# Veason-silverbullet/DIGAT

Hardware: AMD Instinct MI355X
Metric: MIND dev impressions scored/sec (AUC match not run) (higher is better)
Workload: dtype f32; 1 GPU; MIND-small default: --graph_encoder=DIGAT neighbors=3 hops=2 (N=10, U=67), d=400, graph_depth=3, fp32 dev inference; projection=auto -> fp16x3, N=10, U=67, d=400, graph_depth=3, news_num=65238, parallelism=dp1 (row shards, no data-path collective), ranks_in_process_group=1

## Files before the change

### digat_amd/_lib.py

```python
from __future__ import annotations

import ctypes as C
import os
from typing import Optional

import torch

_HERE = os.path.dirname(os.path.abspath(__file__))
LIB_PATH = os.environ.get("DIGAT_HIP_LIB") or os.path.join(_HERE, "lib", "libdigat_hip.so")
DIGAT_MAX_DEPTH = 16
DIGAT_MAX_NODES = 128
GEMM_BF16X6, GEMM_F16X3 = 0, 1
GEMM_F16F8C = 2
PARAMS_GEMM_F16X3 = 64
PARAMS_BD_TILED = 128
PARAMS_PQ_FP8 = 256
PARAMS_SIDE_STREAM_OFF, PARAMS_SIDE_STREAM_ON = 512, 1024
PARAMS_NO_LIVE_ROWS = 2048
PARAMS_PROJ_F16F8C = 4096
PARAMS_RAGGED_OFF, PARAMS_RAGGED_ROWMAJOR = 8192, 16384

_f = C.c_void_p


# ... 34 lines not shown
class Params(C.Structure):
    _fields_ = ([("d", C.c_int32), ("depth", C.c_int32), ("category_num", C.c_int32), ("flags", C.c_int32)]
                + [(k, _f) for k in ("topic_node_embedding", "cand_K", "cand_Q", "cand_bQ",
                                     "news_graph_W", "news_graph_b", "user_news_K", "user_news_Q",
                                     "user_news_bQ", "featureAffine_W", "featureAffine_b",
                                     "userAtt_K", "userAtt_Q", "userAtt_bQ")]
                + [("news", LayerParams * DIGAT_MAX_DEPTH), ("user", LayerParams * DIGAT_MAX_DEPTH)]
                + [(k, _f) for k in ("cand_fold_W", "cand_fold_b", "user_news_fold_W", "user_news_fold_b",
                                     "userAtt_fold_W", "userAtt_fold_b", "featureAffine_wsplit", "cand_fold_wsplit", "gate_wsplit")]
                + [("ctx_wsplit", _f * (DIGAT_MAX_DEPTH + 1)), ("range_flag", _f), ("featureAffine_fsplit", _f)])


class DigatHipError(RuntimeError):
    pass


_lib: Optional[C.CDLL] = None

_SIGNATURES = {
    "digat_version": (C.c_int, []),
    "digat_error_string": (C.c_char_p, [C.c_int]),
    "digat_linear_f32": (C.c_int, [_f, C.c_int64, _f, _f, _f, C.c_int64, C.c_int, C.c_int, C.c_int, _f]),
    "digat_xattn_workspace_bytes": (C.c_size_t, [C.c_int] * 3),
    "digat_xattn_fwd": (C.c_int, [_f] * 12 + [C.c_int] * 3 + [_f, C.c_size_t, _f]),
    "digat_xattn_fwd_mode": (C.c_int, [_f] * 11 + [C.c_int] * 4 + [_f, C.c_size_t, _f]),
    "digat_xattn_fwd_lowprec": (C.c_int, [_f] * 11 + [C.c_int, _f] + [C.c_int] * 4 + [_f, C.c_size_t, _f]),
    "digat_xattn_pairwise_fwd": (C.c_int, [_f] * 8 + [C.c_int] * 3 + [_f]),
    "digat_news_ctx_workspace_bytes": (C.c_size_t, [C.c_int] * 3),
    "digat_news_ctx_fwd": (C.c_int, [_f] * 9 + [C.c_int] * 3 + [_f, C.c_size_t, _f]),
    "digat_user_ctx_workspace_bytes": (C.c_size_t, [C.c_int] * 5),
    "digat_user_ctx_fwd": (C.c_int, [_f] * 14 + [C.c_int] * 5 + [_f, C.c_size_t, _f]),
    "digat_user_ctx_grouped_workspace_bytes": (C.c_size_t, [C.c_int] * 6),
    "digat_user_ctx_fwd_grouped": (C.c_int, [_f] * 15 + [C.c_int] * 6 + [_f, C.c_size_t, _f]),
    "digat_user_nodes_build": (C.c_int, [_f] * 4 + [C.c_long, C.c_long] + [C.c_int] * 3 + [_f]),
    "digat_topic_pool_fwd": (C.c_int, [_f] * 4 + [C.c_int] * 5 + [_f]),
    "digat_encoder_workspace_bytes": (C.c_size_t, [C.c_int] * 6),
    "digat_encoder_fwd": (C.c_int, [C.POINTER(Params)] + [_f] * 10 + [C.c_int] * 3 + [_f, C.c_size_t, _f]),
    "digat_row_logits": (C.c_int, [_f] * 3 + [C.c_int] * 2 + [_f]),
    "digat_profile_pause": (C.c_int, [C.c_int]),
    "digat_set_train_precision": (C.c_int, [C.c_int]),
    "digat_gather_tables": (C.c_int, [C.POINTER(GatherJob), C.c_int, _f]),
    "digat_user_graph_build": (C.c_int, [_f, _f, C.c_long, C.c_int, C.c_int, _f, _f, _f, _f]),
    "digat_negative_sample": (C.c_int, [_f, _f, _f, C.c_long, C.c_int, C.c_uint32, C.c_uint32, _f, _f]),
    "digat_train_batch_ids": (C.c_int, [_f, C.c_long, _f, _f, C.c_long, C.c_int, _f, C.c_long, C.c_int, _f, C.c_long, C.c_int, _f, _f, _f, _f, _f]),
    "digat_profile_live_row_fraction": (C.c_double, []),
    "digat_rank_metrics": (C.c_int, [_f] * 3 + [C.c_int] + [_f] * 4),
    "digat_format_rank_file": (C.c_int64, [_f, _f, C.c_int64, _f, C.c_int64]),
    "digat_topk_segments_workspace_bytes": (C.c_size_t, [C.c_int64, C.c_int64, C.c_int]),
    "digat_topk_segments": (C.c_int, [_f, _f, C.c_int64, C.c_int64, _f, _f, C.c_int, C.c_int, _f, _f, _f, _f, C.c_size_t, _f]),
    "digat_dot_topk_workspace_bytes": (C.c_size_t, [C.c_int64, C.c_int64, C.c_int]),
    "digat_dot_topk": (C.c_int, [_f, _f, _f, C.c_int64, C.c_int64, C.c_int64, C.c_int, _f, C.c_int, C.c_int, _f, _f, _f, _f, C.c_size_t, _f]),
    "digat_dot_scores": (C.c_int, [_f, _f, _f, C.c_int64, C.c_int64, C.c_int64, C.c_int, _f, _f]),
    "digat_shortlist_segments_workspace_bytes": (C.c_size_t, [C.c_int64, C.c_int64, C.c_int]),
    "digat_shortlist_segments": (C.c_int, [_f, _f, C.c_int64, C.c_int64, _f, _f, C.c_int, C.c_int, _f, _f, _f, _f, C.c_size_t, _f]),
    "digat_dot_shortlist_workspace_bytes": (C.c_size_t, [C.c_int64, C.c_int64, C.c_int, C.c_int64]),
    "digat_dot_shortlist": (C.c_int, [_f, _f, _f, C.c_int64, C.c_int64, C.c_int64, C.c_int, _f, C.c_int, C.c_int, C.c_int64, _f, _f, _f, _f,
                                      C.c_size_t, _f]),
    "digat_quantize_rows_i8": (C.c_int, [_f, C.c_int64, C.c_int, C.c_int, _f, _f, _f]),
    "digat_qdot_scores": (C.c_int, [_f] * 5 + [C.c_int64] * 3 + [C.c_int, C.c_int, _f, _f]),
    "digat_qdot_topk_workspace_bytes": (C.c_size_t, [C.c_int64, C.c_int64, C.c_int]),
    "digat_qdot_topk": (C.c_int, [_f] * 5 + [C.c_int64] * 3 + [C.c_int, C.c_int, _f, C.c_int, C.c_int, _f, _f, _f, _f, C.c_size_t, _f]),
    "digat_qdot_shortlist_workspace_bytes": (C.c_size_t, [C.c_int64, C.c_int64, C.c_int, C.c_int64]),
    "digat_qdot_shortlist": (C.c_int, [_f] * 5 + [C.c_int64] * 3 + [C.c_int, C.c_int, _f, C.c_int, C.c_int, C.c_int64, _f, _f, _f, _f,
                                       C.c_size_t, _f]),
    "digat_dot_rank_workspace_bytes":(C.c_size_t, [C.c_int64, C.c_int64, C.c_int64]),
    "digat_dot_rank": (C.c_int, [_f, _f, _f, C.c_int64, C.c_int64, C.c_int64, C.c_int, _f, C.c_int, _f, _f, C.c_int64, _f, _f, _f, C.c_size_t, _f]),
# ... 296 lines not shown
```

### digat_amd/csrc/digat_encoder.inc

```
static size_t max_sz(size_t a, size_t b) { return a > b ? a : b; }

struct FoldCtxWs { float *T, *T2, *glob; };
struct EncoderWs {
    float *Xu[2], *Xn[2];
    char* xws; size_t xws_bytes;
    XattnWs xu;
    char* cws; size_t cws_bytes;
    FoldCtxWs fc;
    float *kq_t, *kq_u, *r_user[2], *r_news;
    char* xws_news; size_t xws_news_bytes;
    XattnWs xn;
    int *cnt, *off, *idx, *cnt2, *off2, *idx2, *entries, *flag, *hlast;
    uint8_t *flags1, *flags2;
    int *cnt_n, *off_n, *idx_n; uint8_t* flags_n;
    int *l0_gs, *l0_off; uint8_t* l0_lead; int* l0_idx;
    unsigned* tw_word; int* tw_list; uint8_t* tw_flags; int *tw_cnt, *tw_off;
    int *gl_off, *gl_idx;
    int* idx32;
    uint8_t *Au, *cm; int64_t* ci;
    uint8_t *fg, *tfg; unsigned* twg; uint8_t* bfg; int *cg, *eg, *hg, *bcg, *tcg;
    uint8_t *same, *is_leader, *lead; int* leader_of;
};
static bool encoder_carve(Arena& a, int B, int N, int H, int C, int d, int variant, EncoderWs& e) {
    const int U = H + C, C1 = C + 1, nmax = N > U ? N : U;
// ... 18 lines not shown
    e.flags1 = a.take<uint8_t>(bu); e.flags2 = a.take<uint8_t>(b * C1);
    e.cnt_n = a.take<int>(b); e.off_n = a.take<int>(b + 1); e.idx_n = a.take<int>(b * N); e.flags_n = a.take<uint8_t>(b * N);
    e.l0_gs = a.take<int>(b + 64); e.l0_off = a.take<int>(b + 64); e.l0_lead = a.take<uint8_t>(b); e.l0_idx = a.take<int>(bu);
    e.tw_word = a.take<unsigned>(bu); e.tw_list = a.take<int>(bu); e.tw_flags = a.take<uint8_t>(bu);
    e.tw_cnt = a.take<int>(b + 64); e.tw_off = a.take<int>(b + 64);
    e.gl_off = a.take<int>(b + 64); e.gl_idx = a.take<int>(bu);
    e.idx32 = a.take<int>(b);
    if (variant == ENC_GROUPED) {
        const size_t g = b / 4 + 1;
        e.Au = a.take<uint8_t>(bu * U); e.cm = a.take<uint8_t>(b * C1); e.ci = a.take<int64_t>(b * H);
        e.fg = a.take<uint8_t>(g * U); e.tfg = a.take<uint8_t>(g * U); e.twg = a.take<unsigned>(g * U); e.bfg = a.take<uint8_t>(g * C1);
        for (int** x : {&e.cg, &e.eg, &e.hg, &e.bcg, &e.tcg}) *x = a.take<int>(g);
    } else if (variant == ENC_SHARED) {
        e.same = a.take<uint8_t>(b); e.is_leader = a.take<uint8_t>(b); e.lead = a.take<uint8_t>(b); e.leader_of = a.take<int>(b);
    }
    return a.ok && xa.ok && ca.ok && na.ok;
}
static size_t encoder_ws_bytes(int B, int N, int H, int C, int d, int variant) { Arena a; EncoderWs e; encoder_carve(a, B, N, H, C, d, variant, e); return a.used; }

struct EncoderCall {
    const digat_params* p;
    const float* Xn_in; const uint8_t *An, *Mn;
    const float* ue;
    const uint8_t *Au, *cat_mask; const int64_t* cat_idx;
    const float* c_n0; float *out_news, *out_user;
    int B, N, H;
    void* workspace; size_t workspace_bytes; hipStream_t st;
    int variant;
    const int* row_group; int G;
    const uint8_t *Au_g, *cm_g; const int64_t* ci_g;
    const float *news_hpq0, *hist_hpq0, *topic_hpq0, *ctxq0; const int64_t* news_index; int64_t news_rows;
    const uint8_t *run_leader, *run_lead;
    EncoderPlan plan;
    EncoderWs ws;
};
struct SideStream { hipStream_t s; hipEvent_t fork, join, early; int ok; };
constexpr int SPARSE_PER_NODE = 20;
static SideStream* side_stream(hipStream_t caller) {
    struct Entry { int dev; hipStream_t caller; SideStream side; int state; };
    static Entry tab[64];
    static int used = 0;
    static std::mutex mu;
    int dev = 0;
    if (hipGetDevice(&dev) != hipSuccess) return nullptr;
    std::lock_guard<std::mutex> lock(mu);
    for (int i = 0; i < used; ++i)
        if (tab[i].dev == dev && tab[i].caller == caller) return tab[i].state == 1 ? &tab[i].side : nullptr;
    if (used == 64) return nullptr;
    Entry& e = tab[used++];
    e.dev = dev; e.caller = caller;
    SideStream& x = e.side;
    const bool ok = hipStreamCreateWithFlags(&x.s, hipStreamNonBlocking) == hipSuccess &&
                    hipEventCreateWithFlags(&x.fork, hipEventDisableTiming) == hipSuccess &&
                    hipEventCreateWithFlags(&x.join, hipEventDisableTiming) == hipSuccess &&
                    hipEventCreateWithFlags(&x.early, hipEventDisableTiming) == hipSuccess;
    e.state = ok ? 1 : -1;
    return ok ? &x : nullptr;
}

static int grid_blocks(long total4, int cap) {
    const int blocks = (int)((total4 + 255) / 256);
    return blocks > cap ? cap : blocks;
}

static GemmArgs ctx_queries_args(const digat_params* p, const float* c_n, int M, int next_layer, float* kq_topic, float* kq_user, float* k3) {
    const GemmFormats f = gemm_formats(p);
// ... 42 lines not shown
    FoldedPass(const EncoderCall& call, const float* Xg0_, SideStream* side_)
        : c(call), pl(call.plan), Xg0(Xg0_), side(side_), p(call.p), w(call.ws), st(call.st), B(call.B), N(call.N), H(call.H), G(call.G),
          d(call.p->d), C(call.p->category_num), L(call.p->depth), U(call.H + call.p->category_num), C1(call.p->category_num + 1),
          f(gemm_formats(call.p)), ragged(encoder_ragged(call.p->flags)), c_n(call.out_news), c_u(call.out_user), c_n_src(call.plan.c_n0_in_place ? call.c_n0 : call.out_news) {}

    int context_queries(int next_layer, hipStream_t sq) const {
        return launch_gemm(ctx_queries_args(p, next_layer == 0 ? c_n_src : c_n, B, next_layer, w.kq_t, w.kq_u, w.r_user[next_layer & 1]), sq);
    }

    int user_context(const float* Xu_cur, const float* addend, hipStream_t sq, const int* xgroup, bool lists,
                     const float* kq_topic = nullptr, const float* kq_user = nullptr) const {
        if (!kq_topic) { kq_topic = w.kq_t; kq_user = w.kq_u; }
        const uint8_t* flags = lists ? live.flags : nullptr;
        const int* hist_last = flags ? live.hist_last : nullptr;
        if (pl.user_ctx_fused) {
            const CtxFusedArgs fa{Xu_cur, (long)U * d, xgroup, flags, U, hist_last, kq_topic, kq_user, c.cat_idx, c.cat_mask, addend, c_u,
                                  (const uint4*)p->featureAffine_fsplit, p->featureAffine_b, f.range_flag, B, H, C1, d, sqrtf((float)d)};
            return launch_user_ctx_fused(fa, sq);
        }
        float *T = w.fc.T, *T2 = w.fc.T2;
        int e = launch_topic(Xu_cur, (long)U * d, kq_topic, c.cat_idx, T, B, H, C1, d, sq, xgroup, flags, U, hist_last);
        if (e) return e;
        GemmArgs g = gemm_plain(T, d, p->featureAffine_W, p->featureAffine_b, T2, d, B * C1, d, d, 0);
        g.epi = EPI_RELU_RES; g.e0 = T; g.lde0 = d;
        g.wsplit = (const unsigned short*)p->featureAffine_wsplit;
        g.format = f.fmt; g.range_flag = f.range_flag;
        g.ragged = ragged;
        if (live.bucket_idx && gemm_takes_row_list(g)) { g.rowidx = live.bucket_idx; g.nrows_dev = live.nbuckets; }
        e = launch_gemm(g, sq);
        if (e) return e;
        return launch_pool(T2, (long)C1 * d, kq_user, c.cat_mask, addend, c_u, B, C1, d, sq);
    }

    int news_context(const float* Xn_cur, hipStream_t sq, bool first) const {
        const long ldx = (long)N * d;
        float *kq = w.kq_t, *glob = w.fc.glob;
        GemmArgs gq = gemm_plain(Xn_cur, ldx, p->cand_fold_W, p->cand_fold_b, kq, d, B, d, d, 0);
        gq.wsplit = (const unsigned short*)p->cand_fold_wsplit; gq.format = f.fmt; gq.range_flag = f.range_flag;
        gq.m_dispatch = pl.bd_disp;
        int e = launch_gemm(gq, sq);
        if (e) return e;
        e = launch_pool(Xn_cur, ldx, kq, c.Mn, nullptr, glob, B, N, d, sq);
        if (e) return e;
        GemmArgs g = gemm_plain(Xn_cur, ldx, p->news_graph_W, p->news_graph_b, c_n, d, B, d, 2 * d, 0);
        g.k0 = d; g.a1 = glob; g.lda1 = d;
        g.epi = EPI_GATE; g.e0 = Xn_cur; g.lde0 = ldx; g.e1 = glob; g.lde1 = d; g.e2 = first ? c_n_src : c_n; g.lde2 = d;
        g.wsplit = (const unsigned short*)p->gate_wsplit; g.format = f.fmt; g.range_flag = f.range_flag;
        g.m_dispatch = 1;
        return launch_gemm(g, sq);
    }

    int live_flags(const LiveFlagsJob& j, const LiveArrays& rows, hipStream_t sq) const {
        const bool want_entries = pl.sparse_mode == DIGAT_XATTN_AUTO, twins = pl.twins;
        const LiveArrays& o = j.out;
        hipLaunchKernelGGL(user_live_flags_kernel, dim3((j.rows + 3) / 4), dim3(256), (size_t)4 * ((U * U + 63) & ~63), sq, j.Au, j.cat_mask, j.cat_idx,
                           j.rows, U, H, C1, o.flags, o.cnt, want_entries ? o.entries : (int*)nullptr, o.hlast, o.bflags, o.bcnt,
                           twins ? o.twin : (unsigned*)nullptr, twins ? o.tflags : (uint8_t*)nullptr, twins ? o.tcnt : (int*)nullptr, j.rowmask);
        DIGAT_CHECK_LAUNCH();
        if (!j.expand) return DIGAT_OK;
        LiveExpand le;
        le.flags_g = o.flags; le.twin_g = twins ? o.twin : nullptr; le.tflags_g = o.tflags; le.bflags_g = o.bflags;
        le.cnt_g = o.cnt; le.entries_g = o.entries; le.hlast_g = o.hlast; le.bcnt_g = o.bcnt; le.tcnt_g = o.tcnt;
        le.flags = rows.flags; le.twin = twins ? rows.twin : nullptr; le.tflags = rows.tflags; le.bflags = rows.bflags;
        le.cnt = rows.cnt; le.entries = want_entries ? rows.entries : nullptr; le.hlast = rows.hlast; le.bcnt = rows.bcnt;
        le.tcnt = twins ? rows.tcnt : nullptr;
        hipLaunchKernelGGL(live_expand_kernel, dim3((B + 3) / 4), dim3(256), 0, sq, le, c.row_group, B, U, C1);
// ... 202 lines not shown
    }

    static bool record(hipEvent_t e, hipStream_t s) { return hipEventRecord(e, s) == hipSuccess; }
    static bool wait(hipStream_t s, hipEvent_t e) { return hipStreamWaitEvent(s, e, 0) == hipSuccess; }

    int run() {
        int rc;
        const bool group_early = side && L > 0 && pl.by_group;
        const bool live_early = side && pl.want_scan;
        if (side && (pl.news_early || group_early || live_early)) {
            if (!record(side->fork, st) || !wait(side->s, side->fork)) return DIGAT_ERR_LAUNCH;
        }
        if (live_early) {
            rc = adjacency_pass(side->s);
            if (rc) return rc;
        }
        if (group_early) {
            rc = group_projection(side->s);
            if (rc) return rc;
        }
        if (group_early || live_early) {
            if (!record(side->early, side->s)) return DIGAT_ERR_LAUNCH;
        }
        if (pl.news_early && !pl.news_cached0) {
            rc = news_projection(0, c.Xn_in, side ? side->s : st);
            if (rc) return rc;
        }
        const size_t bd = (size_t)B * d;
        const float* const ctxq0 = pl.ctxq0 ? c.ctxq0 : nullptr;
        if (!ctxq0) {
            rc = context_queries(0, st);
            if (rc) return rc;
        }
        rc = user_context(pl.xu0_grouped ? Xg0 : w.Xu[0], nullptr, st, (pl.xu0_grouped || pl.xu0_shared) ? c.row_group : nullptr, false,
                          ctxq0, ctxq0 ? ctxq0 + bd : nullptr);
        if (rc) return rc;
        const float* xn_cur = c.Xn_in;
        int un = 0, nn = 0;
        for (int i = 0; i < L; ++i) {
            const float* r_user = (i == 0 && ctxq0) ? ctxq0 + 2 * bd : w.r_user[i & 1];
            hipStream_t sn = side ? side->s : st;
            if (side && i == 0) {
                if (!record(side->fork, st) || !wait(sn, side->fork)) return DIGAT_ERR_LAUNCH;
            }
            if (side && i > 0) {
                if (!wait(st, side->join)) return DIGAT_ERR_LAUNCH;
            }
            if (i == 0 && pl.want_scan && !live_early) {
                rc = adjacency_pass(st);
                if (rc) return rc;
            }
            if (i == 0 && side && (group_early || live_early)) {
                if (!wait(st, side->early)) return DIGAT_ERR_LAUNCH;
            }
            if (i == 0 && pl.want_live) publish();
            rc = (i == 0 && pl.by_group) ? user_layer0_grouped(r_user, group_early) : user_layer(i, r_user, w.Xu[un], w.Xu[un ^ 1]);
            if (rc) return rc;
            if (side && !record(side->fork, st)) return DIGAT_ERR_LAUNCH;
            rc = news_k3(i, sn);
            if (rc) return rc;
            if (i == 0 && pl.news_lists) {
                rc = news_live_lists(sn);
                if (rc) return rc;
            }
            rc = news_layer(i, xn_cur, w.Xn[nn], sn);
            if (rc) return rc;
            xn_cur = w.Xn[nn]; nn ^= 1; un ^= 1;
            rc = news_context(xn_cur, sn, i == 0);
// ... 62 lines not shown
        o.wsplit = ln.wsplit;
        rc = xattn_core(xn_cur, c.An, w.r_news, ln.W, ln.bW, ln.F1, ln.F2, ln.a, w.Xn[nn], nullptr, B, N, d, w.xws, w.xws_bytes, st, o);
        if (rc) return rc;
        rc = launch_gemm(gemm_plain(c.out_news, d, lu.F3, lu.b3, w.r_user[0], d, B, d, d, 0), st);
        if (rc) return rc;
        o.wsplit = lu.wsplit;
        rc = xattn_core(w.Xu[un], c.Au, w.r_user[0], lu.W, lu.bW, lu.F1, lu.F2, lu.a, w.Xu[un ^ 1], nullptr, B, U, d, w.xws, w.xws_bytes, st, o);
        if (rc) return rc;
        xn_cur = w.Xn[nn]; nn ^= 1; un ^= 1;
        rc = digat_news_ctx_fwd(xn_cur, c.Mn, p->cand_K, p->cand_Q, p->cand_bQ, p->news_graph_W, p->news_graph_b,
                                c.out_news, c.out_news, B, N, d, w.cws, w.cws_bytes, st);
        if (rc) return rc;
        rc = digat_user_ctx_fwd(w.Xu[un], c.cat_mask, c.cat_idx, c.out_news, p->user_news_K, p->user_news_Q, p->user_news_bQ,
                                p->featureAffine_W, p->featureAffine_b, p->userAtt_K, p->userAtt_Q, p->userAtt_bQ,
                                c.out_user, c.out_user, B, U, H, C + 1, d, w.cws, w.cws_bytes, st);
        if (rc) return rc;
    }
    return DIGAT_OK;
}

static int encoder_fwd_impl(EncoderCall& c) {
    const digat_params* p = c.p;
    const bool grouped = c.variant == ENC_GROUPED;
    if (!p || !c.Xn_in || !c.An || !c.Mn || !c.ue || !c.out_news || !c.out_user || !c.workspace) return DIGAT_ERR_ARG;
    if (grouped ? (!c.Au_g || !c.cm_g || !c.ci_g || !c.row_group) : (!c.Au || !c.cat_mask || !c.cat_idx)) return DIGAT_ERR_ARG;
    const int B = c.B, N = c.N, H = c.H, G = c.G, d = p->d, C = p->category_num, U = H + C;
    EncoderPlanIn in = {};
    in.flags = p->flags; in.B = B; in.N = N; in.H = H; in.C = C; in.d = d; in.L = p->depth; in.G = G; in.variant = c.variant;
    in.folded = p->cand_fold_W && p->user_news_fold_W && p->userAtt_fold_W;
    in.c_n0 = c.c_n0; in.news_hpq0 = c.news_hpq0; in.hist_hpq0 = c.hist_hpq0; in.topic_hpq0 = c.topic_hpq0; in.ctxq0 = c.ctxq0;
    in.news_index = c.news_index; in.news_rows = c.news_rows;
    in.fsplit = p->featureAffine_fsplit; in.ctx_fused_fits = ctxfused_ok(H, C + 1, d);
    const EncoderPlan& pl = c.plan = encoder_plan(in);
    if (pl.status) return pl.status;
    Arena ar(c.workspace, c.workspace_bytes);
    if (!encoder_carve(ar, B, N, H, C, d, c.variant, c.ws)) return DIGAT_ERR_WORKSPACE;
    if (B == 0) return DIGAT_OK;
    if (pl.status_after_carve) return pl.status_after_carve;
    hipStream_t st = c.st;
    const EncoderWs& w = c.ws;
    int rc = encoder_user_rows(c);
    if (rc) return rc;
    float* const Xg0 = pl.xu0_grouped ? w.xu.h + 2 * (size_t)G * U * d : nullptr;
    {
        const long nrows = pl.xu0_grouped ? G : B;
        ProfScope prof(DIGAT_KERNEL_GLUE, (double)nrows * ((double)H * d * 8 + (double)C * d * 4), st);
        hipLaunchKernelGGL(build_user_nodes_kernel, dim3(grid_blocks(nrows * U * (d / 4), 2048)), dim3(256), 0, st, (const float4*)c.ue,
                           (const float4*)p->topic_node_embedding, (float4*)(pl.xu0_grouped ? Xg0 : w.Xu[0]), nrows, H, C, d / 4,
                           (pl.xu0_grouped || pl.shared) ? (const int*)nullptr : c.row_group, pl.shared ? c.run_leader : (const uint8_t*)nullptr);
        DIGAT_CHECK_LAUNCH();
    }
    if (pl.c_n0_in_place) {
    } else if (c.c_n0) {
        if (hipMemcpyAsync(c.out_news, c.c_n0, (size_t)B * d * 4, hipMemcpyDeviceToDevice, st) != hipSuccess)
            return DIGAT_ERR_LAUNCH;
    } else {
        rc = digat_news_ctx_fwd(c.Xn_in, c.Mn, p->cand_K, p->cand_Q, p->cand_bQ, p->news_graph_W, p->news_graph_b,
                                nullptr, c.out_news, B, N, d, w.cws, w.cws_bytes, st);
        if (rc) return rc;
    }
    if (!pl.folded) return encoder_fwd_unfolded(c);
    return FoldedPass(c, Xg0, pl.side_wanted ? side_stream(st) : nullptr).run();
}

int digat_encoder_fwd(const digat_params* p, const float* Xn_in, const uint8_t* An, const uint8_t* Mn,
                      const float* ue, const uint8_t* Au, const uint8_t* cat_mask, const int64_t* cat_idx,
// ... 78 lines not shown
```

### digat_amd/csrc/digat_encoder_plan.h

```cpp
#pragma once
#include <stddef.h>
#include <stdint.h>
#include "../../include/digat_hip.h"
#include "digat_xattn_plan.h"

enum { ENC_PLAIN, ENC_GROUPED, ENC_SHARED };

struct GemmFormats { int fmt, lfmt; unsigned* range_flag; };
static inline GemmFormats gemm_formats(int flags, void* range_flag) {
    const int fmt = (flags & DIGAT_PARAMS_GEMM_F16X3) ? 1 : 0;
    return GemmFormats{fmt, (flags & DIGAT_PARAMS_PROJ_F16F8C) ? DIGAT_GEMM_F16F8C : fmt, fmt ? (unsigned*)range_flag : nullptr};
}
static inline GemmFormats gemm_formats(const digat_params* p) { return gemm_formats(p->flags, p->range_flag); }
static inline int bd_dispatch(int flags) { return (flags & DIGAT_PARAMS_BD_TILED) ? (1 << 30) : 1; }

struct EncoderPlanIn {
    int flags, B, N, H, C, d, L, G, variant;
    bool folded;
    bool c_n0, news_hpq0, hist_hpq0, topic_hpq0, ctxq0, news_index; int64_t news_rows;
    bool fsplit;
    bool ctx_fused_fits;
};

struct EncoderPlan {
    int status;
    int status_after_carve;
    bool folded;
    bool shared;
    bool by_group;
    bool xu0_grouped;
    bool xu0_shared;
    bool c_n0_in_place;
    bool ctxq0;
    int sparse_mode;
    bool want_live, want_scan;
    bool l0_chunked, twins;
    bool l0_sparse, l0_dense;
    bool group_tables;
    int pq_x3, pq_mode;
    int fmt, lfmt, bd_disp;
    bool news_early;
    bool news_lists;
    int news_sparse_mode;
    bool news_cached0, news_indexed0;
    bool user_ctx_fused;
    int side_mode;
    bool side_wanted;
};

static inline EncoderPlan encoder_plan(const EncoderPlanIn& in) {
    EncoderPlan pl = {};
    const int flags = in.flags, B = in.B, N = in.N, H = in.H, C = in.C, d = in.d, L = in.L, U = H + C;
    const bool grouped = in.variant == ENC_GROUPED, folded = in.folded;
    pl.status = pl.status_after_carve = DIGAT_OK;
    pl.folded = folded;
    if (in.hist_hpq0 != in.topic_hpq0) { pl.status = DIGAT_ERR_ARG; return pl; }
    if (in.ctxq0 && !in.c_n0) { pl.status = DIGAT_ERR_ARG; return pl; }
    if (grouped && in.G <= 0) { pl.status = DIGAT_ERR_ARG; return pl; }
    if (B < 0 || N <= 0 || H < 0) { pl.status = DIGAT_ERR_ARG; return pl; }
    if (grouped && !folded) { pl.status = DIGAT_ERR_ARG; return pl; }
    if (d <= 0 || d % 4 || L < 0 || L > DIGAT_MAX_DEPTH || N > DIGAT_MAX_NODES || U > DIGAT_MAX_NODES || C < 0) { pl.status = DIGAT_ERR_SHAPE; return pl; }
    if (grouped && (size_t)4 * in.G > (size_t)B) { pl.status = DIGAT_ERR_SHAPE; return pl; }
    if (in.news_index && !(in.c_n0 && in.news_hpq0 && L > 0 && eq8_row_fits_wave(d) && in.news_rows > 0 && in.news_rows <= 0x7fffffffLL &&
                           (eq8_small_graph(N) || ((flags & DIGAT_NEWS_XATTN_SPARSE) && N <= DIGAT_MAX_NODES)) && folded))
        pl.status_after_carve = DIGAT_ERR_ARG;

    pl.shared = in.variant == ENC_SHARED && folded && L > 0 && (flags & 3) == DIGAT_XATTN_SPARSE && !(flags & DIGAT_PARAMS_NO_LIVE_ROWS) &&
                eq8_multi_centre_fits(d, U) && eq8_sparse_graph(U);
    pl.by_group = grouped || pl.shared;
    pl.xu0_grouped = grouped && folded && L > 0 && (flags & 3) == DIGAT_XATTN_SPARSE && eq8_row_fits_wave(d) && eq8_sparse_graph(U) && 3 * (long)in.G <= B;
    pl.c_n0_in_place = in.c_n0 && folded && L > 0;
    pl.ctxq0 = folded && in.ctxq0 && in.c_n0;
    const GemmFormats f = gemm_formats(flags, nullptr);
    pl.fmt = f.fmt; pl.lfmt = f.lfmt; pl.bd_disp = bd_dispatch(flags);
    pl.pq_x3 = (flags & DIGAT_PROJ_PQ_X3) ? 1 : 0;
    pl.pq_mode = ((flags & DIGAT_PQ_BF16) ? 1 : 0) | ((flags & DIGAT_PQ_X1) ? 2 : 0) | ((flags & DIGAT_PQ_FP8) ? 4 : 0);
    pl.sparse_mode = flags & 3;
    if (pl.sparse_mode == 3 || (pl.sparse_mode == DIGAT_XATTN_AUTO && L == 0)) pl.sparse_mode = DIGAT_XATTN_DENSE;
    pl.xu0_shared = pl.shared && pl.sparse_mode == DIGAT_XATTN_SPARSE;
    pl.want_live = L > 0 && !(flags & DIGAT_PARAMS_NO_LIVE_ROWS);
    pl.want_scan = pl.want_live || pl.sparse_mode == DIGAT_XATTN_AUTO;
// ... 20 lines not shown
```

### digat_amd/csrc/digat_kernels.hip

```cpp
#include <hip/hip_runtime.h>
#include <stdint.h>
#include <string.h>
#include <stdlib.h>
#include <atomic>
#include <initializer_list>
#include <mutex>
#include <type_traits>
#include <unordered_map>
#include <utility>

#include "../../include/digat_hip.h"
#include "digat_encoder_plan.h"
#include "digat_xattn_plan.h"

typedef float v4f __attribute__((ext_vector_type(4)));

#define DIGAT_CHECK_LAUNCH()                                   \
    do {                                                       \
        if (hipGetLastError() != hipSuccess) return DIGAT_ERR_LAUNCH; \
    } while (0)

static inline size_t align_up(size_t v, size_t a) { return (v + a - 1) / a * a; }
struct Arena {
    char* base; size_t cap, used; bool ok;
// ... 110 lines not shown
    __builtin_amdgcn_s_waitcnt((N & 15) | (7 << 4) | (15 << 8) | ((N >> 4) << 14));
}
__device__ __forceinline__ void wait_vmcnt(int n) {
    switch (n) {
        case 0: asm volatile("s_waitcnt vmcnt(0)" ::: "memory"); break;
        case 1: asm volatile("s_waitcnt vmcnt(1)" ::: "memory"); break;
        case 2: asm volatile("s_waitcnt vmcnt(2)" ::: "memory"); break;
        case 3: asm volatile("s_waitcnt vmcnt(3)" ::: "memory"); break;
        case 4: asm volatile("s_waitcnt vmcnt(4)" ::: "memory"); break;
        case 5: asm volatile("s_waitcnt vmcnt(5)" ::: "memory"); break;
        case 6: asm volatile("s_waitcnt vmcnt(6)" ::: "memory"); break;
        default: asm volatile("s_waitcnt vmcnt(4)" ::: "memory"); break;
    }
}

__device__ __forceinline__ float leaky02_uniform(float e) {
    const float t = 0.2f * e;
    float r;
    asm("v_max_f32 %0, %1, %2" : "=v"(r) : "s"(e), "v"(t));
    return r;
}
__host__ __device__ __forceinline__ unsigned hash32(unsigned x) {
    x ^= x >> 16; x *= 0x7feb352dU; x ^= x >> 15; x *= 0x846ca68bU; x ^= x >> 16;
    return x;
}
__host__ __device__ __forceinline__ unsigned drop_threshold(float p) { return (unsigned)(p * 4294967296.0); }
__device__ __forceinline__ bool drop_keep(unsigned seed, long e, unsigned thr) {
    return hash32((unsigned)e * 0x9E3779B9U + hash32(seed + (unsigned)(e >> 32))) >= thr;
}
constexpr int TWIN_R = DIGAT_TWIN_R;
#include "digat_gemm.inc"
#include "digat_xattn.inc"
#include "digat_context.inc"
#include "digat_ctxfused.inc"
#include "digat_glue.inc"

extern "C" {

int digat_version(void) { return DIGAT_ABI_VERSION; }

const char* digat_error_string(int code) {
    switch (code) {
        case DIGAT_OK: return "ok";
        case DIGAT_ERR_ARG: return "bad argument (null pointer or negative size)";
        case DIGAT_ERR_SHAPE: return "unsupported shape (d % 4 != 0, graph larger than DIGAT_MAX_NODES, depth too large)";
        case DIGAT_ERR_WORKSPACE: return "workspace too small";
        case DIGAT_ERR_LAUNCH: return "HIP kernel launch failed";
        default: return "unknown error";
    }
}

int digat_linear_f32(const float* x, int64_t ldx, const float* w, const float* b, float* y, int64_t ldy,
                     int M, int N, int K, void* stream) {
    if (!x || !w || !y || M < 0 || N <= 0 || K <= 0) return DIGAT_ERR_ARG;
    if (K % 4 || ldx % 4) return DIGAT_ERR_SHAPE;
    return launch_gemm(gemm_plain(x, ldx, w, b, y, ldy, M, N, K, 0), (hipStream_t)stream);
}

struct XattnWs { float *h, *P, *Q, *r, *alpha; };
static XattnWs xattn_carve(Arena& a, int B, int n, int d) {
    const size_t nd = (size_t)B * n * d;
    XattnWs w{};
    w.h = a.take<float>(3 * nd);
    if (w.h) { w.P = w.h + nd; w.Q = w.P + nd; }
    w.r = a.take<float>((size_t)B * d);
    w.alpha = a.take<float>((size_t)B * n * n);
// ... 366 lines not shown
    float *qv = w.qv, *kq = w.kq, *T = w.T, *T2 = w.T2;
    int rc;
    rc = launch_gemm(gemm_plain(c_n, d, Qu, bQu, qv, d, B, d, d, 0), st);
    if (rc) return rc;
    rc = launch_gemm(gemm_plain(qv, d, Ku, nullptr, kq, d, B, d, d, 1), st);
    if (rc) return rc;
    rc = launch_topic(Xu, (long)U * d, kq, cat_idx, T, B, H, C1, d, st, group);
    if (rc) return rc;
    GemmArgs g = gemm_plain(T, d, Fa, bFa, T2, d, B * C1, d, d, 0);
    g.epi = EPI_RELU_RES; g.e0 = T; g.lde0 = d;
    rc = launch_gemm(g, st);
    if (rc) return rc;
    rc = launch_gemm(gemm_plain(c_n, d, Qua, bQua, qv, d, B, d, d, 0), st);
    if (rc) return rc;
    rc = launch_gemm(gemm_plain(qv, d, Kua, nullptr, kq, d, B, d, d, 1), st);
    if (rc) return rc;
    return launch_pool(T2, (long)C1 * d, kq, cat_mask, addend, out, B, C1, d, st);
}

int digat_user_ctx_fwd(const float* Xu, const uint8_t* cat_mask, const int64_t* cat_idx, const float* c_n,
                       const float* Ku, const float* Qu, const float* bQu, const float* Fa, const float* bFa,
                       const float* Kua, const float* Qua, const float* bQua, const float* addend, float* out,
                       int B, int U, int H, int C1, int d, void* workspace, size_t workspace_bytes, void* stream) {
    if (!Xu || !cat_mask || !cat_idx || !c_n || !Ku || !Qu || !Fa || !Kua || !Qua || !out || !workspace)
        return DIGAT_ERR_ARG;
    if (B < 0 || H < 0 || U < H || C1 <= 0 || d <= 0) return DIGAT_ERR_ARG;
    if (d % 4 || C1 > DIGAT_MAX_NODES || H > TOPIC_MAX_H) return DIGAT_ERR_SHAPE;
    Arena ar(workspace, workspace_bytes);
    const UserCtxWs w = user_ctx_carve(ar, B, C1, d);
    if (!ar.ok) return DIGAT_ERR_WORKSPACE;
    if (B == 0) return DIGAT_OK;
    return user_ctx_run(Xu, cat_mask, cat_idx, nullptr, c_n, Ku, Qu, bQu, Fa, bFa, Kua, Qua, bQua, addend, out, B, U, H, C1, d, w,
                        (hipStream_t)stream);
}

__global__ void __launch_bounds__(256) transpose_kernel(const float* __restrict__ in, float* __restrict__ out, int d) {
    __shared__ float tile[32][33];
    const int bx = blockIdx.x * 32, by = blockIdx.y * 32;
    for (int r = threadIdx.y; r < 32; r += 8) {
        const int y = by + r, x = bx + threadIdx.x;
        if (y < d && x < d) tile[r][threadIdx.x] = in[(long)y * d + x];
    }
    __syncthreads();
    for (int r = threadIdx.y; r < 32; r += 8) {
        const int y = bx + r, x = by + threadIdx.x;
        if (y < d && x < d) out[(long)y * d + x] = tile[threadIdx.x][r];
    }
}

size_t digat_fold_workspace_bytes(int d) { return 2 * align_up((size_t)d * d * 4, 256); }

int digat_fold_attention(const float* K, const float* Q, const float* bQ, float* Wf, float* bf, int d,
                         void* workspace, size_t workspace_bytes, void* stream) {
    if (!K || !Q || !Wf || !bf || !workspace || d <= 0) return DIGAT_ERR_ARG;
    if (d % 4) return DIGAT_ERR_SHAPE;
    if (workspace_bytes < digat_fold_workspace_bytes(d)) return DIGAT_ERR_WORKSPACE;
    hipStream_t st = (hipStream_t)stream;
    float* Kt = (float*)workspace;
    float* Qt = (float*)((char*)workspace + align_up((size_t)d * d * 4, 256));
    const dim3 grid((d + 31) / 32, (d + 31) / 32), block(32, 8);
    hipLaunchKernelGGL(transpose_kernel, grid, block, 0, st, K, Kt, d);
    hipLaunchKernelGGL(transpose_kernel, grid, block, 0, st, Q, Qt, d);
    DIGAT_CHECK_LAUNCH();
    int rc = launch_gemm(gemm_plain(Kt, d, Qt, nullptr, Wf, d, d, d, d, 0), st);
    if (rc) return rc;
    if (bQ) return launch_gemm(gemm_plain(bQ, d, Kt, nullptr, bf, d, 1, d, d, 0), st);
// ... 149 lines not shown
```

### include/digat_hip.h

```cpp
#ifndef DIGAT_HIP_H
#define DIGAT_HIP_H

#include <stddef.h>
#include <stdint.h>

#ifdef __cplusplus
extern "C" {
#endif

#define DIGAT_ABI_VERSION 4
#define DIGAT_MAX_NODES 128
#define DIGAT_MAX_DEPTH 16

enum {
    DIGAT_OK = 0,
    DIGAT_ERR_ARG = 1,
    DIGAT_ERR_SHAPE = 2,
    DIGAT_ERR_WORKSPACE = 3,
    DIGAT_ERR_LAUNCH = 4
};

int digat_version(void);
const char* digat_error_string(int code);

// ... 26 lines not shown
int digat_xattn_fwd_lowprec(const float* X, const uint8_t* A, const float* ctx,
                            const float* W, const float* bW, const float* F1, const float* F2,
                            const float* F3, const float* b3, const float* a, const void* wsplit, int format,
                            float* out, int B, int n, int d, int pq,
                            void* workspace, size_t workspace_bytes, void* stream);

int digat_xattn_pairwise_fwd(const float* Pr, const float* Q, const float* h, const float* X,
                             const float* a, const uint8_t* A,
                             float* out, float* alpha, int B, int n, int d, void* stream);

size_t digat_news_ctx_workspace_bytes(int B, int N, int d);
int digat_news_ctx_fwd(const float* X, const uint8_t* mask,
                       const float* Kc, const float* Qc, const float* bQc,
                       const float* Wg, const float* bg,
                       const float* addend, float* out, int B, int N, int d,
                       void* workspace, size_t workspace_bytes, void* stream);

size_t digat_user_ctx_workspace_bytes(int B, int U, int H, int C1, int d);
int digat_user_ctx_fwd(const float* Xu, const uint8_t* cat_mask, const int64_t* cat_idx, const float* c_n,
                       const float* Ku, const float* Qu, const float* bQu,
                       const float* Fa, const float* bFa,
                       const float* Kua, const float* Qua, const float* bQua,
                       const float* addend, float* out, int B, int U, int H, int C1, int d,
                       void* workspace, size_t workspace_bytes, void* stream);

size_t digat_user_ctx_grouped_workspace_bytes(int B, int G, int U, int H, int C1, int d);
int digat_user_ctx_fwd_grouped(const float* Xu, const uint8_t* cat_mask, const int64_t* cat_idx, const int32_t* row_group,
                               const float* c_n,
                               const float* Ku, const float* Qu, const float* bQu,
                               const float* Fa, const float* bFa,
                               const float* Kua, const float* Qua, const float* bQua,
                               const float* addend, float* out, int B, int G, int U, int H, int C1, int d,
                               void* workspace, size_t workspace_bytes, void* stream);

int digat_user_nodes_build(const float* ue, const float* topic, const int32_t* row_group, float* Xu, long rows, long G, int H,
                           int C, int d, void* stream);

int digat_topic_pool_fwd(const float* Xu, const float* kq, const int64_t* cat_idx, float* out,
                         int B, int U, int H, int C1, int d, void* stream);

enum { DIGAT_XATTN_AUTO = 0, DIGAT_XATTN_DENSE = 1, DIGAT_XATTN_SPARSE = 2 };
enum { DIGAT_PROJ_PQ_X3 = 4 };
enum { DIGAT_NEWS_XATTN_SPARSE = 8 };
enum { DIGAT_PQ_BF16 = 16, DIGAT_PQ_X1 = 32 };
enum { DIGAT_PQ_FP8 = 256 };
enum { DIGAT_PARAMS_GEMM_F16X3 = 64 };
enum { DIGAT_PARAMS_BD_TILED = 128 };

typedef struct digat_layer_params {
    const float *W, *bW;
    const float *F1;
    const float *F2;
    const float *F3, *b3;
    const float *a;
    const void  *wsplit;
    const void  *f3_wsplit;
} digat_layer_params;

typedef struct digat_params {
    int32_t d;
    int32_t depth;
    int32_t category_num;
    int32_t flags;
    const float *topic_node_embedding;
    const float *cand_K, *cand_Q, *cand_bQ;
    const float *news_graph_W, *news_graph_b;
// ... 450 lines not shown
```

Measured before the change: 38350 impressions/s.

## Add fused layer-0 user context kernel using linearity of feature affine

Adds a specialised layer-0 user-context path. It runs the feature-affine GEMM once on the raw history embeddings (rows*H rather than B*C1 topic rows). A single per-row kernel then does topic attention, topic pooling with MFMA, ReLU-residual, user attention pooling and the output. This relies on the pooled-topic affine being linear, so affine(pool(x)) = pool(affine(x)) before bias. It replaces the separate topic, GEMM and pool launches, at the cost of a larger GEMM when histories outnumber topics and heavy LDS and register use.

```diff
diff --git a/digat_amd/_lib.py b/digat_amd/_lib.py
--- a/digat_amd/_lib.py
+++ b/digat_amd/_lib.py
@@ -90,6 +90,7 @@
     "digat_user_ctx_fwd": (C.c_int, [_f] * 14 + [C.c_int] * 5 + [_f, C.c_size_t, _f]),
     "digat_user_ctx_grouped_workspace_bytes": (C.c_size_t, [C.c_int] * 6),
     "digat_user_ctx_fwd_grouped": (C.c_int, [_f] * 15 + [C.c_int] * 6 + [_f, C.c_size_t, _f]),
+    "digat_user_ctx0_fwd": (C.c_int, [_f, _f, C.c_int] + [_f] * 7 + [C.c_int, _f, _f] + [C.c_int] * 4 + [_f, C.c_size_t, _f]),
     "digat_user_nodes_build": (C.c_int, [_f] * 4 + [C.c_long, C.c_long] + [C.c_int] * 3 + [_f]),
     "digat_topic_pool_fwd": (C.c_int, [_f] * 4 + [C.c_int] * 5 + [_f]),
     "digat_encoder_workspace_bytes": (C.c_size_t, [C.c_int] * 6),
diff --git a/digat_amd/csrc/digat_ctx0.inc b/digat_amd/csrc/digat_ctx0.inc
--- /dev/null
+++ b/digat_amd/csrc/digat_ctx0.inc
@@ -0,0 +1,200 @@
+struct Ctx0Args {
+    const float* x; const float* fx; long ld_b;
+    const int* group;
+    const float *kq_topic, *kq_user;
+    const int64_t* idx; const uint8_t* mask;
+    const float *bias, *addend; float* out;
+    int B, H, C1, d; float sqrt_d;
+};
+
+template <int CTX0_STEPS>
+__global__ void __launch_bounds__(CTX0_STEPS > 13 ? 512 : 1024, CTX0_STEPS > 13 ? 1 : 5) user_ctx0_kernel(const Ctx0Args g) {
+    extern __shared__ __attribute__((aligned(16))) unsigned char smem[];
+    const int H = g.H, hs = H | 1, C1 = g.C1, d = g.d;
+    const int ct = (C1 + 15) >> 4;
+    const int tid = threadIdx.x, lane = tid & 63, wave = tid >> 6;
+    const int nthreads = blockDim.x, nw = nthreads >> 6;
+    float* M = reinterpret_cast<float*>(smem);
+    float* part = M + ct * 16 * hs;
+    float* sa = part + nw * 64;
+    int* sidx = reinterpret_cast<int*>(sa + 64);
+    int* cslot = sidx + 64;
+    int* scat = cslot + 64;
+    float* pe = reinterpret_cast<float*>(scat + 68);
+    float* Tl = pe + 16;
+    const int b = blockIdx.x;
+    const long gb = (long)(g.group ? g.group[b] : b) * g.ld_b;
+    const float* Xb = g.x + gb;
+    const float* Fb = g.fx + gb;
+    const int lr = lane & 15, lq = lane >> 4;
+    const int ch = wave * 64 + 4 * lr;
+    const bool ch_ok = ch < d;
+    const int nsteps = (H + 3) >> 2;
+
+    float4 xq[CTX0_STEPS];
+#pragma unroll
+    for (int s = 0; s < CTX0_STEPS; ++s) {
+        const int j = s * 4 + lq;
+        xq[s] = (s < nsteps && j < H && ch_ok) ? *reinterpret_cast<const float4*>(Xb + (long)j * d + ch) : f4_zero();
+    }
+    const float4 k4 = ch_ok ? *reinterpret_cast<const float4*>(g.kq_topic + (long)b * d + ch) : f4_zero();
+    if (tid < 64) {
+        long v = -1;
+        if (tid < H) v = g.idx[(long)b * H + tid];
+        const unsigned long long mb = __ballot(tid < C1 && g.mask[(long)b * C1 + min(tid, C1 - 1)] != 0);
+        const int cat = (v >= 0 && v < C1 && (mb == 0ull || ((mb >> v) & 1ull))) ? (int)v : -1;
+        sidx[tid] = cat;
+        unsigned long long present = 0ull;
+        for (int c = 0; c < C1; ++c) present |= __ballot(cat == c) ? (1ull << c) : 0ull;
+        const bool has = tid < C1 && ((present >> tid) & 1ull);
+        const int slot = __popcll(present & ((1ull << tid) - 1ull));
+        cslot[tid] = has ? slot : -1;
+        if (has) scat[slot] = tid;
+        const unsigned long long used = __ballot(cat >= 0);
+        if (tid == 0) { scat[64] = __popcll(present); scat[65] = used ? 64 - __clzll(used) : 0; }
+    }
+    for (int i = tid; i < ct * 16 * hs; i += nthreads) M[i] = 0.f;
+
+#pragma unroll
+    for (int s = 0; s < CTX0_STEPS; ++s) {
+        float p = fmaf(xq[s].w, k4.w, fmaf(xq[s].z, k4.z, fmaf(xq[s].y, k4.y, xq[s].x * k4.x)));
+        p += dpp_mov<0xB1>(p); p += dpp_mov<0x4E>(p); p += dpp_mov<0x141>(p); p += dpp_mov<0x140>(p);
+        if (lr == 0) part[wave * 64 + s * 4 + lq] = p;
+    }
+    __syncthreads();
+    if (tid < 64) {
+        float a = 0.f;
+        for (int w = 0; w < nw; ++w) a += part[w * 64 + tid];
+        sa[tid] = a / g.sqrt_d;
+    }
+    __syncthreads();
+    {
+        const int my = lane < H ? sidx[lane] : -2;
+        const float v = lane < H ? sa[lane] : 0.f;
+        const int nslots = scat[64];
+        for (int sl = wave; sl < nslots; sl += nw) {
+            const int c = scat[sl];
+            const bool in = my == c;
+            const float m = wave_max(in ? v : -INFINITY);
+            const float e = in ? expf(v - m) : 0.f;
+            const float den = wave_sum(e);
+            if (in) M[sl * hs + lane] = e / den;
+        }
+    }
+    __syncthreads();
+
+    const int nslots = scat[64];
+    const int ct_eff = __builtin_amdgcn_readfirstlane((nslots + 15) >> 4);
+    const int nl = __builtin_amdgcn_readfirstlane(scat[65]);
+    for (int it = 0; it < ct_eff; ++it) {
+        const bool last = it == ct_eff - 1;
+        v4f acc[4];
+#pragma unroll
+        for (int s = 0; s < 4; ++s) acc[s] = (v4f){0.f, 0.f, 0.f, 0.f};
+#pragma unroll
+        for (int s = 0; s < CTX0_STEPS; ++s) {
+            if (s * 4 < nl) {
+                const int j = s * 4 + lq;
+                const float4 xc = xq[s];
+                const float av = j < H ? M[(it * 16 + lr) * hs + j] : 0.f;
+                acc[0] = __builtin_amdgcn_mfma_f32_16x16x4f32(av, xc.x, acc[0], 0, 0, 0);
+                acc[1] = __builtin_amdgcn_mfma_f32_16x16x4f32(av, xc.y, acc[1], 0, 0, 0);
+                acc[2] = __builtin_amdgcn_mfma_f32_16x16x4f32(av, xc.z, acc[2], 0, 0, 0);
+                acc[3] = __builtin_amdgcn_mfma_f32_16x16x4f32(av, xc.w, acc[3], 0, 0, 0);
+                if (last) xq[s] = (j < H && ch_ok) ? *reinterpret_cast<const float4*>(Fb + (long)j * d + ch) : f4_zero();
+            }
+        }
+#pragma unroll
+        for (int r = 0; r < 4; ++r) {
+            const int sl = it * 16 + 4 * lq + r;
+            if (sl < nslots && ch_ok)
+                *reinterpret_cast<float4*>(Tl + (long)sl * d + ch) = make_float4(acc[0][r], acc[1][r], acc[2][r], acc[3][r]);
+        }
+    }
+    const float4 b4 = ch_ok ? *reinterpret_cast<const float4*>(g.bias + ch) : f4_zero();
+    const float4 ku4 = ch_ok ? *reinterpret_cast<const float4*>(g.kq_user + (long)b * d + ch) : f4_zero();
+    for (int it = 0; it < ct_eff; ++it) {
+        v4f acc[4];
+#pragma unroll
+        for (int s = 0; s < 4; ++s) acc[s] = (v4f){0.f, 0.f, 0.f, 0.f};
+#pragma unroll
+        for (int s = 0; s < CTX0_STEPS; ++s) {
+            if (s * 4 < nl) {
+                const int j = s * 4 + lq;
+                const float4 xc = xq[s];
+                const float av = j < H ? M[(it * 16 + lr) * hs + j] : 0.f;
+                acc[0] = __builtin_amdgcn_mfma_f32_16x16x4f32(av, xc.x, acc[0], 0, 0, 0);
+                acc[1] = __builtin_amdgcn_mfma_f32_16x16x4f32(av, xc.y, acc[1], 0, 0, 0);
+                acc[2] = __builtin_amdgcn_mfma_f32_16x16x4f32(av, xc.z, acc[2], 0, 0, 0);
+                acc[3] = __builtin_amdgcn_mfma_f32_16x16x4f32(av, xc.w, acc[3], 0, 0, 0);
+            }
+        }
+#pragma unroll
+        for (int r = 0; r < 4; ++r) {
+            const int sl = it * 16 + 4 * lq + r;
+            float p = 0.f;
+            if (sl < nslots && ch_ok) {
+                float4* tp = reinterpret_cast<float4*>(Tl + (long)sl * d + ch);
+                const float4 t = *tp;
+                const float4 v = make_float4(fmaxf(acc[0][r] + b4.x, 0.f) + t.x, fmaxf(acc[1][r] + b4.y, 0.f) + t.y,
+                                             fmaxf(acc[2][r] + b4.z, 0.f) + t.z, fmaxf(acc[3][r] + b4.w, 0.f) + t.w);
+                *tp = v;
+                p = fmaf(v.w, ku4.w, fmaf(v.z, ku4.z, fmaf(v.y, ku4.y, v.x * ku4.x)));
+            }
+            p += dpp_mov<0xB1>(p); p += dpp_mov<0x4E>(p); p += dpp_mov<0x141>(p); p += dpp_mov<0x140>(p);
+            if (lr == 0 && sl < nslots) part[wave * 64 + sl] = p;
+        }
+    }
+    const float4 e4 = make_float4(fmaxf(b4.x, 0.f), fmaxf(b4.y, 0.f), fmaxf(b4.z, 0.f), fmaxf(b4.w, 0.f));
+    {
+        float p = fmaf(e4.w, ku4.w, fmaf(e4.z, ku4.z, fmaf(e4.y, ku4.y, e4.x * ku4.x)));
+        p += dpp_mov<0xB1>(p); p += dpp_mov<0x4E>(p); p += dpp_mov<0x141>(p); p += dpp_mov<0x140>(p);
+        if (lane == 0) pe[wave] = p;
+    }
+    __syncthreads();
+    float v = -INFINITY;
+    if (lane < C1) {
+        const int sl = cslot[lane];
+        float a = 0.f;
+        for (int w = 0; w < nw; ++w) a += sl >= 0 ? part[w * 64 + sl] : pe[w];
+        v = g.mask[(long)b * C1 + lane] == 0 ? -1e9f : a / g.sqrt_d;
+    }
+    const float m = wave_max(v);
+    const float e = lane < C1 ? expf(v - m) : 0.f;
+    const float den = wave_sum(e);
+    const float al = e / den;
+    float4 o = f4_zero();
+    for (int c = 0; c < C1; ++c) {
+        const float a = lane_bcast(al, c);
+        if (a == 0.f) continue;
+        const int sl = cslot[c];
+        const float4 t2 = sl < 0 ? e4 : (ch_ok ? *reinterpret_cast<const float4*>(Tl + (long)sl * d + ch) : f4_zero());
+        o.x = fmaf(a, t2.x, o.x); o.y = fmaf(a, t2.y, o.y); o.z = fmaf(a, t2.z, o.z); o.w = fmaf(a, t2.w, o.w);
+    }
+    if (lq == 0 && ch_ok) {
+        if (g.addend) o = f4_add(*reinterpret_cast<const float4*>(g.addend + (long)b * d + ch), o);
+        *reinterpret_cast<float4*>(g.out + (long)b * d + ch) = o;
+    }
+}
+
+static int launch_user_ctx0(const float* ue, long rows, const int* group, const float* kq_topic, const float* kq_user,
+                            const int64_t* idx, const uint8_t* mask, const float* Fa, const float* bFa, const void* wsplit, int format,
+                            unsigned* range_flag, int ragged, const float* addend, float* out, float* fx, int B, int H, int C1, int d,
+                            hipStream_t st) {
+    if (!ctx0_fits(H, C1, d) || rows <= 0 || rows * H > 0x7fffffffL) return DIGAT_ERR_SHAPE;
+    if (B == 0) return DIGAT_OK;
+    GemmArgs gf = gemm_plain(ue, d, Fa, nullptr, fx, d, (int)(rows * H), d, d, 0);
+    gf.wsplit = (const unsigned short*)wsplit; gf.format = format; gf.range_flag = range_flag;
+    gf.m_dispatch = 1 << 30;
+    gf.ragged = ragged ? ragged : DIGAT_GEMM_RAGGED;
+    int rc = launch_gemm(gf, st);
+    if (rc) return rc;
+    const Ctx0Args g{ue, fx, (long)H * d, group, kq_topic, kq_user, idx, mask, bFa, addend, out, B, H, C1, d, sqrtf((float)d)};
+    ProfScope prof(DIGAT_KERNEL_TOPIC, (double)rows * H * d * 8.0 + (double)B * (3.0 * d * 4 + H * 8.0 + C1), st);
+    const int groups = (d + 63) / 64;
+    const size_t lds = ctx0_lds_bytes(H, C1, d);
+    if (H <= 52) hipLaunchKernelGGL(user_ctx0_kernel<13>, dim3(B), dim3(64 * groups), lds, st, g);
+    else hipLaunchKernelGGL(user_ctx0_kernel<16>, dim3(B), dim3(64 * groups), lds, st, g);
+    DIGAT_CHECK_LAUNCH();
+    return DIGAT_OK;
+}
diff --git a/digat_amd/csrc/digat_encoder.inc b/digat_amd/csrc/digat_encoder.inc
--- a/digat_amd/csrc/digat_encoder.inc
+++ b/digat_amd/csrc/digat_encoder.inc
@@ -74,6 +74,7 @@
     const float *news_hpq0, *hist_hpq0, *topic_hpq0, *ctxq0; const int64_t* news_index; int64_t news_rows;
     const uint8_t *run_leader, *run_lead;
     EncoderPlan plan;
+    bool ctx0;
     EncoderWs ws;
 };
 struct SideStream { hipStream_t s; hipEvent_t fork, join, early; int ok; };
@@ -182,6 +183,15 @@
         return launch_pool(T2, (long)C1 * d, kq_user, c.cat_mask, addend, c_u, B, C1, d, sq);
     }
 
+    int user_context0(const float* kq_topic, const float* kq_user) const {
+        if (!kq_topic) { kq_topic = w.kq_t; kq_user = w.kq_u; }
+        const bool per_group = c.variant == ENC_GROUPED;
+        float* const fx = w.Xu[1] + (per_group ? (size_t)G * U * d : 0);
+        return launch_user_ctx0(c.ue, per_group ? G : B, (per_group || pl.shared) ? c.row_group : nullptr, kq_topic, kq_user, c.cat_idx,
+                                c.cat_mask, p->featureAffine_W, p->featureAffine_b, p->featureAffine_wsplit, f.fmt, f.range_flag, ragged,
+                                nullptr, c_u, fx, B, H, C1, d, st);
+    }
+
     int news_context(const float* Xn_cur, hipStream_t sq, bool first) const {
         const long ldx = (long)N * d;
         float *kq = w.kq_t, *glob = w.fc.glob;
@@ -450,8 +460,9 @@
             rc = context_queries(0, st);
             if (rc) return rc;
         }
-        rc = user_context(pl.xu0_grouped ? Xg0 : w.Xu[0], nullptr, st, (pl.xu0_grouped || pl.xu0_shared) ? c.row_group : nullptr, false,
-                          ctxq0, ctxq0 ? ctxq0 + bd : nullptr);
+        rc = c.ctx0 ? user_context0(ctxq0, ctxq0 ? ctxq0 + bd : nullptr)
+                    : user_context(pl.xu0_grouped ? Xg0 : w.Xu[0], nullptr, st, (pl.xu0_grouped || pl.xu0_shared) ? c.row_group : nullptr, false,
+                                   ctxq0, ctxq0 ? ctxq0 + bd : nullptr);
         if (rc) return rc;
         const float* xn_cur = c.Xn_in;
         int un = 0, nn = 0;
@@ -580,6 +591,7 @@
     in.news_index = c.news_index; in.news_rows = c.news_rows;
     in.fsplit = p->featureAffine_fsplit; in.ctx_fused_fits = ctxfused_ok(H, C + 1, d);
     const EncoderPlan& pl = c.plan = encoder_plan(in);
+    c.ctx0 = encoder_plan_ctx0(in);
     if (pl.status) return pl.status;
     Arena ar(c.workspace, c.workspace_bytes);
     if (!encoder_carve(ar, B, N, H, C, d, c.variant, c.ws)) return DIGAT_ERR_WORKSPACE;
diff --git a/digat_amd/csrc/digat_encoder_plan.h b/digat_amd/csrc/digat_encoder_plan.h
--- a/digat_amd/csrc/digat_encoder_plan.h
+++ b/digat_amd/csrc/digat_encoder_plan.h
@@ -47,6 +47,16 @@
     int side_mode;
     bool side_wanted;
 };
+
+static inline size_t ctx0_lds_bytes(int H, int C1, int d) {
+    const size_t ct = (size_t)(C1 + 15) / 16, waves = (size_t)(d + 63) / 64;
+    return (ct * 16 * (size_t)(H | 1) + waves * 64 + 3 * 64 + 68 + 16 + (size_t)C1 * d) * 4;
+}
+static inline bool ctx0_fits(int H, int C1, int d) {
+    return H >= 1 && H <= 64 && d > 0 && d % 4 == 0 && d <= 1024 && C1 >= 1 && C1 <= 64 && (H <= 52 || d <= 512) &&
+           ctx0_lds_bytes(H, C1, d) <= (size_t)64 * 1024;
+}
+static inline bool encoder_plan_ctx0(const EncoderPlanIn& in) { return in.folded && ctx0_fits(in.H, in.C + 1, in.d); }
 
 static inline EncoderPlan encoder_plan(const EncoderPlanIn& in) {
     EncoderPlan pl = {};
diff --git a/digat_amd/csrc/digat_kernels.hip b/digat_amd/csrc/digat_kernels.hip
--- a/digat_amd/csrc/digat_kernels.hip
+++ b/digat_amd/csrc/digat_kernels.hip
@@ -166,6 +166,7 @@
 #include "digat_gemm.inc"
 #include "digat_xattn.inc"
 #include "digat_context.inc"
+#include "digat_ctx0.inc"
 #include "digat_ctxfused.inc"
 #include "digat_glue.inc"
 
@@ -598,6 +599,20 @@
     if (B == 0) return DIGAT_OK;
     return user_ctx_run(Xu, cat_mask, cat_idx, nullptr, c_n, Ku, Qu, bQu, Fa, bFa, Kua, Qua, bQua, addend, out, B, U, H, C1, d, w,
                         (hipStream_t)stream);
+}
+
+int digat_user_ctx0_fwd(const float* ue, const int32_t* row_group, int G, const float* kq_topic, const float* kq_user,
+                        const uint8_t* cat_mask, const int64_t* cat_idx, const float* Fa, const float* bFa,
+                        const void* fa_wsplit, int format, const float* addend, float* out, int B, int H, int C1, int d,
+                        void* scratch, size_t scratch_bytes, void* stream) {
+    if (!ue || !kq_topic || !kq_user || !cat_mask || !cat_idx || !Fa || !bFa || !out || !scratch) return DIGAT_ERR_ARG;
+    if (B < 0 || H < 0 || C1 <= 0 || d <= 0 || (row_group && G <= 0)) return DIGAT_ERR_ARG;
+    if (!ctx0_fits(H, C1, d)) return DIGAT_ERR_SHAPE;
+    const long rows = row_group ? G : B;
+    if (scratch_bytes < (size_t)rows * H * d * 4) return DIGAT_ERR_WORKSPACE;
+    if (B == 0) return DIGAT_OK;
+    return launch_user_ctx0(ue, rows, row_group, kq_topic, kq_user, cat_idx, cat_mask, Fa, bFa, fa_wsplit, format, nullptr, 0, addend, out,
+                            (float*)scratch, B, H, C1, d, (hipStream_t)stream);
 }
 
 __global__ void __launch_bounds__(256) transpose_kernel(const float* __restrict__ in, float* __restrict__ out, int d) {
diff --git a/include/digat_hip.h b/include/digat_hip.h
--- a/include/digat_hip.h
+++ b/include/digat_hip.h
@@ -82,6 +82,11 @@
                                const float* Kua, const float* Qua, const float* bQua,
                                const float* addend, float* out, int B, int G, int U, int H, int C1, int d,
                                void* workspace, size_t workspace_bytes, void* stream);
+
+int digat_user_ctx0_fwd(const float* ue, const int32_t* row_group, int G, const float* kq_topic, const float* kq_user,
+                        const uint8_t* cat_mask, const int64_t* cat_idx, const float* Fa, const float* bFa,
+                        const void* fa_wsplit, int format, const float* addend, float* out, int B, int H, int C1, int d,
+                        void* scratch, size_t scratch_bytes, void* stream);
 
 int digat_user_nodes_build(const float* ue, const float* topic, const int32_t* row_group, float* Xu, long rows, long G, int H,
                            int C, int d, void* stream);
```

Result: faster. 39180 impressions/s, median of 6 (+2.2%).
